# Crispy13/GeneFuseRust

Measured on NVIDIA B200. Metric: read_pairs_per_sec_matched, higher is better.
Workload: dtype u8/int64

## Files before the change

### genefuserust_b200/csrc/gf_api.cu

```cuda
#include <algorithm>
#include <chrono>
#include <cstdlib>
#include <condition_variable>
#include <cstring>
#include <mutex>
#include <thread>

#include "gf_internal.h"

static thread_local std::string g_last_error;
void gf_set_error(const std::string& msg) { g_last_error = msg; }

__global__ void k_fill_uniform(uint64_t* off, uint32_t* pko, uint64_t base, uint32_t len, uint64_t n) {
    const uint64_t i = (uint64_t)blockIdx.x * blockDim.x + threadIdx.x;
    if (i <= n) off[i] = base + i * len;
    if (i < n) pko[i] = (uint32_t)(i * 2u * ((len + 31u) >> 5));
}

namespace {

constexpr uint64_t CHUNK_TARGET_BYTES = 192ull << 20;

int fail(int code, const std::string& msg) {
    gf_set_error(msg);
// ... 33 lines not shown
        uint64_t mx = 0;
        bool b = false;
        for (uint64_t i = n * t / nt; i < n * (t + 1) / nt; i++) {
            const uint64_t a = off1[i], e = off1[i + 1];
            b |= e < a;
            mx = std::max(mx, e - a);
            if (off2) {
                const uint64_t a2 = off2[i], e2 = off2[i + 1];
                b |= e2 < a2;
                mx = std::max(mx, e2 - a2);
            }
        }
        part[t] = mx;
        bad[t] = b;
    };
    if (nt == 1) work(0);
    else {
        std::vector<std::thread> th;
        for (unsigned t = 0; t < nt; t++) th.emplace_back(work, t);
        for (auto& x : th) x.join();
    }
    uint64_t mx = 0;
    for (unsigned t = 0; t < nt; t++) {
        if (bad[t]) return fail(GF_E_INVALID, "offsets are not ascending");
        mx = std::max(mx, part[t]);
    }
    if (mx > limit) return fail(GF_E_INVALID, "a read is longer than the kernel capacity (max_len hint too small, or > 1024 bases)");
    *max_len = mx;
    return GF_OK;
}

void destroy_handle(gf_index* idx) {
    if (!idx) return;
    cudaSetDevice(idx->device);
    if (idx->busy && idx->ev_busy) cudaEventSynchronize(idx->ev_busy);
    if (idx->stream) cudaStreamSynchronize(idx->stream);
    if (idx->copy_stream) cudaStreamSynchronize(idx->copy_stream);
    cudaFree(idx->d_table);
    cudaFree(idx->d_dupes);
    cudaFree(idx->d_gene_ascii);
    cudaFree(idx->d_gene_start);
    cudaFree(idx->d_gene_len);
    cudaFree(idx->d_gene_rev);
    cudaFree(idx->d_planes);
    cudaFree(idx->d_filter);
    cudaFree(idx->d_granule);
    idx->ws_survivors.release();
    idx->ws_counters.release();
    idx->ws_gtbl.release();
    idx->ws_seq_words.release();
    idx->ws_seq_meta.release();
    idx->ws_seq_seed.release();
    idx->ws_seq_lists.release();
    idx->fq[0].release();
    idx->fq[1].release();
    idx->bgzf_comp[0].release(); idx->bgzf_comp[1].release();
    idx->bgzf_members[0].release(); idx->bgzf_members[1].release();
    idx->bgzf_status.release();
    for (auto& s : idx->stage) {
        s.seq1.release(); s.qual1.release(); s.off1.release();
        s.seq2.release(); s.qual2.release(); s.off2.release();
        s.out.release(); s.nout.release(); s.out2.release(); s.keys.release();
        for (int m = 0; m < 2; m++) {
            s.pk[m].release(); s.pko[m].release(); s.pkx[m].release(); s.pxo[m].release();
        }
        if (s.copied) cudaEventDestroy(s.copied);
        if (s.done) cudaEventDestroy(s.done);
    }
    for (auto& ps : idx->pack_set) {
        for (int m = 0; m < 2; m++) { ps.h_pk[m].release(); ps.h_pko[m].release(); ps.h_pkx[m].release(); ps.h_pxo[m].release(); }
        if (ps.copied) cudaEventDestroy(ps.copied);
    }
    if (idx->h_slots) cudaFreeHost(idx->h_slots);
    for (cudaEvent_t e : {idx->ev_start, idx->ev_end, idx->ev_ingest})
        if (e) cudaEventDestroy(e);
    for (GfChunkEvents& ce : idx->chunk_events)
        for (cudaEvent_t e : ce.e)
            if (e) cudaEventDestroy(e);
    if (idx->stream) cudaStreamDestroy(idx->stream);
    if (idx->copy_stream) cudaStreamDestroy(idx->copy_stream);
    if (idx->ev_busy) cudaEventDestroy(idx->ev_busy);
    delete idx;
}

}

extern "C" {

const char* gf_last_error(void) { return g_last_error.c_str(); }
int gf_abi_version(void) { return GF_ABI_VERSION; }

int gf_device_count(void) {
    int n = 0;
    if (cudaGetDeviceCount(&n) != cudaSuccess) {
        cudaGetLastError();
        return 0;
    }
    return n;
}

void gf_default_params(gf_params* p) {
    p->skip_key_dup_threshold = 5;
    p->major_gene_key_requirement = 40;
    p->minor_gene_key_requirement = 20;
    p->mismatch_threshold = 10;
    p->deletion_threshold = 50;
// ... 1137 lines not shown
```

### genefuserust_b200/csrc/gf_internal.h

```cpp
#pragma once
#include <cuda_runtime.h>

#include <mutex>
#include <string>
#include <vector>

#include "../../include/genefuse_gpu.h"
#include "gf_device.cuh"
#include "gf_pack.h"

void gf_set_error(const std::string& msg);

#define GF_CUDA_TRY(expr)                                                                              \
    do {                                                                                               \
        cudaError_t _e = (expr);                                                                       \
        if (_e != cudaSuccess) {                                                                       \
            gf_set_error(std::string(#expr) + " failed: " + cudaGetErrorString(_e) + " (" + __FILE__ + \
                         ":" + std::to_string(__LINE__) + ")");                                        \
            return GF_E_CUDA;                                                                          \
        }                                                                                              \
    } while (0)

struct GfBuf {
    void* p = nullptr;
// ... 77 lines not shown

struct GfFastqTable {
    uint64_t n_records = 0;
    uint32_t max_len = 0;
    GfBuf nl, s, e, qs;
    GfBuf cnt, off, tmp;
    void release() { nl.release(); s.release(); e.release(); qs.release(); cnt.release(); off.release(); tmp.release(); }
};

struct GfChunkEvents {
    cudaEvent_t e[6] = {nullptr, nullptr, nullptr, nullptr, nullptr, nullptr};
};

struct GfBgzfMember {
    uint64_t in_off;
    uint64_t out_off;
    uint32_t clen, isize, crc, pad;
};
int gf_bgzf_inflate_device(const uint8_t* d_comp, const GfBgzfMember* d_members, uint32_t n, uint8_t* d_text, unsigned int* d_status,
                           cudaStream_t st);
struct GfFastqMembers {
    const uint8_t* comp = nullptr;
    uint64_t comp_bytes = 0;
    const GfBgzfMember* members = nullptr;
    uint32_t n_members = 0;
    uint64_t text_bytes = 0;
};

struct gf_index {
    int device = 0;
    gf_params params{};
    GfDevIndex dev{};
    gf_index_info info{};
    uint32_t n_genes = 0;
    std::vector<uint32_t> gene_start, gene_len;

    void *d_table = nullptr, *d_dupes = nullptr, *d_gene_ascii = nullptr, *d_gene_start = nullptr,
         *d_gene_len = nullptr, *d_gene_rev = nullptr, *d_planes = nullptr, *d_filter = nullptr, *d_granule = nullptr;

    std::mutex mu;
    cudaStream_t stream = nullptr, copy_stream = nullptr;
    cudaEvent_t ev_busy = nullptr;
    bool busy = false;
    cudaEvent_t ev_start = nullptr, ev_end = nullptr;
    cudaEvent_t ev_ingest = nullptr;
    std::vector<GfChunkEvents> chunk_events;
    uint32_t n_chunks_timed = 0;
    bool split_events = false;
    bool ev_valid = false;

    GfBuf ws_survivors, ws_counters, ws_gtbl;
    GfFastqTable fq[2];
    GfBuf ws_seq_words, ws_seq_meta, ws_seq_seed, ws_seq_lists;
    GfStage stage[GF_STAGES];
    GfPackSet pack_set[GF_PACK_SETS];
    GfBuf bgzf_comp[2], bgzf_members[2], bgzf_status;
    GfHostSlot* h_slots = nullptr;
    bool stats_pending = false;
    uint64_t pending_pairs = 0;
    gf_map_stats stats{};
    unsigned long long launches = 0;
    int sm_count = 148;
    uint32_t out_mode = 0;
};

int gf_build_index_device(gf_index* idx, const gf_gene_span* genes, uint32_t n_genes);
int gf_lookup_device(gf_index* idx, const uint32_t* kmers, uint64_t n, gf_lookup* out);

size_t gf_scan_tmp_elems(uint64_t n);
cudaError_t gf_exclusive_scan_u32(const uint32_t* in, uint32_t* out, uint64_t n, uint32_t* tmp, cudaStream_t st);

int gf_fastq_parse_device(const uint8_t* d_text, uint64_t bytes, GfFastqTable* out, cudaStream_t st, bool final_chunk = true);
int gf_map_fastq_text(gf_index* idx, const uint8_t* fq1, uint64_t bytes1, const uint8_t* fq2, uint64_t bytes2, bool final_chunk,
                      gf_match* out, uint64_t out_cap, uint64_t* n_out, uint64_t* n_records, uint64_t consumed[2],
                      const GfFastqMembers* members = nullptr );
int gf_fastq_fetch_text(gf_index* idx, int k, uint64_t from, uint64_t len, uint8_t* dst);

struct GfDevBatch {
    uint64_t n;
    const uint8_t *seq1, *qual1, *seq2, *qual2;
    const uint64_t *s1, *e1, *qs1, *s2, *e2, *qs2;
    uint64_t base1, base2;
    uint64_t bytes1, bytes2;
    uint64_t pair_base;
    uint32_t max_len;
    const uint32_t *pk1 = nullptr, *pk2 = nullptr;
    const uint32_t *pko1 = nullptr, *pko2 = nullptr;
    const uint32_t *pkx1 = nullptr, *pkx2 = nullptr;
    const uint32_t *pxo1 = nullptr, *pxo2 = nullptr;
};
int gf_map_device_batch(gf_index* idx, const GfDevBatch& b, gf_match* d_out, uint64_t out_cap,
                        unsigned long long* d_n_out, cudaStream_t stream, GfChunkEvents* ev, bool first,
                        gf_index* store_owner = nullptr);
int gf_map_device_batches(gf_index* const* hs, uint32_t nh, const GfDevBatch& b, gf_match* const* d_outs, uint64_t out_cap,
                          unsigned long long* const* d_n_outs, cudaStream_t stream);
int gf_finish_records_device(gf_index* idx, const gf_match* d_in, const unsigned long long* d_n_in, uint64_t in_cap,
                             gf_match* d_out2, unsigned long long* d_keys, unsigned long long* d_n_out2, uint32_t mode,
                             cudaStream_t stream);
int gf_fast_merge_device(gf_index* idx, const GfDevBatch& b, gf_merge_info* d_out, cudaStream_t stream);
int gf_adjust_break_device(gf_index* idx, const uint8_t* d_bytes, const gf_break_ref* d_refs, const gf_break_job* d_jobs,
                           uint64_t n_jobs, gf_break_out* d_out, unsigned int* d_n_undefined, cudaStream_t stream);
```

### genefuserust_b200/csrc/gf_map.cu

```cuda
#include <climits>
#include <cstdlib>
#include <cstdio>

#include "gf_internal.h"
#include "gf_swar.cuh"

namespace {

#define FULL 0xFFFFFFFFu
using swar::zero_bytes;

__device__ __forceinline__ uint32_t fsr(const uint32_t* plane, uint32_t bitpos) {
    uint32_t w = bitpos >> 5;
    return __funnelshift_r(plane[w], plane[w + 1], bitpos & 31u);
}
__device__ __forceinline__ uint32_t lowmask(int nbits) {
    return nbits >= 32 ? 0xFFFFFFFFu : ((1u << nbits) - 1u);
}
__device__ __forceinline__ bool record_ok(uint64_t s, uint64_t e, uint64_t base, uint64_t bytes, int max_len) {
    if (e < s || e - s > (uint64_t)max_len || s < base) return false;
    return bytes == 0 || (s - base <= bytes && e - s <= bytes - (s - base));
}

template <int MAXW>
// ... 1230 lines not shown

int gf_map_device_batch(gf_index* idx, const GfDevBatch& b, gf_match* d_out, uint64_t out_cap,
                        unsigned long long* d_n_out, cudaStream_t st, GfChunkEvents* ev, bool first, gf_index* store_owner) {
    const bool record_events = ev != nullptr;
    if (ev)
        for (cudaEvent_t& e : ev->e)
            if (!e) GF_CUDA_TRY(cudaEventCreate(&e));
    const bool paired = b.seq2 != nullptr;
    if (b.n > 0xFFFFFFFFull) {
        gf_set_error("batch too large (n > 2^32-1 pairs): split it");
        return GF_E_LIMIT;
    }
    const uint64_t surv_cap64 = (paired ? 2 : 1) * b.n + 1;
    const uint32_t surv_cap = (uint32_t)(surv_cap64 > 0xFFFFFFFFull ? 0xFFFFFFFFull : surv_cap64);
    GF_CUDA_TRY(idx->ws_survivors.reserve(sizeof(uint2) * (size_t)surv_cap));
    GF_CUDA_TRY(idx->ws_counters.reserve(sizeof(GfMapCounters)));
    GfMapCounters* d_cnt = idx->ws_counters.as<GfMapCounters>();
    if (first) {
        GF_CUDA_TRY(cudaMemsetAsync(d_cnt, 0, sizeof(GfMapCounters), st));
        GF_CUDA_TRY(cudaMemsetAsync(d_n_out, 0, sizeof(unsigned long long), st));
    } else {
        k_roll_counters<<<1, 1, 0, st>>>(d_cnt, d_n_out, out_cap);
    }
    if (record_events) { GF_CUDA_TRY(cudaEventRecord(ev->e[0], st)); idx->split_events = false; }

    const int need_major = (idx->params.major_gene_key_requirement + 1) / 2;
    const int need_minor = (idx->params.minor_gene_key_requirement + 1) / 2;
    ScreenParams sp;
    sp.ix = idx->dev;
    sp.b = b;
    sp.survivors = idx->ws_survivors.as<uint2>();
    sp.survivors_cap = surv_cap;
    sp.counters = d_cnt;
    sp.need_total = need_major + need_minor;
    sp.need_minor = need_minor;

    if (b.n) {
        const int threads = 256, warps = threads / 32;
        const bool small = b.max_len != 0 && b.max_len <= 256;
        const size_t smem = (small ? sizeof(ScreenWarp<8>) : sizeof(ScreenWarp<32>)) * warps;
        const int blocks_per_sm = 3;
        uint64_t want = (b.n + warps - 1) / warps;
        unsigned grid = (unsigned)std::min<uint64_t>(want, (uint64_t)idx->sm_count * blocks_per_sm);
        if (small) {
            const bool w5 = b.max_len <= 160;
            const int NW3 = w5 ? split::SL<5>::NW3 : split::SL<8>::NW3;
            const uint32_t cap = surv_cap;
            const size_t groups = ((size_t)cap + 31) / 32;
            gf_index* own = store_owner ? store_owner : idx;
            if (!store_owner) {
                GF_CUDA_TRY(idx->ws_seq_words.reserve(groups * NW3 * 32 * sizeof(uint32_t)));
                GF_CUDA_TRY(idx->ws_seq_meta.reserve((size_t)cap * sizeof(uint4)));
            }
            GF_CUDA_TRY(idx->ws_seq_seed.reserve((size_t)cap * sizeof(uint2)));
            GF_CUDA_TRY(idx->ws_seq_lists.reserve((size_t)cap * sizeof(uint32_t) + 64));
            split::SeqStore ss;
            ss.words = own->ws_seq_words.as<uint32_t>();
            ss.meta = own->ws_seq_meta.as<uint4>();
            ss.seed = idx->ws_seq_seed.as<uint2>();
            ss.counters = idx->ws_seq_lists.as<unsigned int>();
            ss.list = idx->ws_seq_lists.as<uint32_t>() + 16;
            ss.cap = cap;
            GF_CUDA_TRY(cudaMemsetAsync(ss.counters, 0, 64, st));
            if (store_owner) {
                const unsigned int* oc = store_owner->ws_seq_lists.as<unsigned int>();
                GF_CUDA_TRY(cudaMemcpyAsync(ss.counters, oc, sizeof(unsigned int), cudaMemcpyDeviceToDevice, st));
                GF_CUDA_TRY(cudaMemcpyAsync(ss.counters + 5, oc + 5, sizeof(unsigned int), cudaMemcpyDeviceToDevice, st));
            }
            split::PrepParams pp;
            pp.b = b;
            pp.st = ss;
            pp.counters = d_cnt;
            const size_t psm = sizeof(uint32_t) * tpp::WARPS * (w5 ? tpp::Lay<5>::NWORDS : tpp::Lay<8>::NWORDS) * 32;
            const uint64_t want_b = (b.n + tpp::WARPS * 32 - 1) / (tpp::WARPS * 32);
#define GF_LAUNCH_PREP2(WW, PE, PK)                                                        \
    do {                                                                                   \
        GF_CUDA_TRY(set_smem(split::k_prep<WW, PE, PK>, psm));                             \
        const unsigned pgrid = (unsigned)std::min<uint64_t>(                               \
            want_b, (uint64_t)idx->sm_count * resident_blocks(split::k_prep<WW, PE, PK>, tpp::WARPS * 32, psm)); \
        split::k_prep<WW, PE, PK><<<pgrid, tpp::WARPS * 32, psm, st>>>(pp);                \
    } while (0)
#define GF_LAUNCH_PREP(WW, PE) do { if (b.pk1) GF_LAUNCH_PREP2(WW, PE, true); else GF_LAUNCH_PREP2(WW, PE, false); } while (0)
            if (!store_owner) {
                if (w5) { if (paired) GF_LAUNCH_PREP(5, true); else GF_LAUNCH_PREP(5, false); }
                else { if (paired) GF_LAUNCH_PREP(8, true); else GF_LAUNCH_PREP(8, false); }
            }
#undef GF_LAUNCH_PREP2
#undef GF_LAUNCH_PREP
            if (record_events) GF_CUDA_TRY(cudaEventRecord(ev->e[1], st));
            split::SeedParams sdp;
            sdp.ix = idx->dev;
            sdp.st = ss;
            sdp.need_total = sp.need_total;
            sdp.need_minor = sp.need_minor;
            split::ClassParams cp;
            cp.ix = idx->dev;
            cp.st = ss;
            cp.survivors = sp.survivors;
            cp.survivors_cap = sp.survivors_cap;
            cp.counters = d_cnt;
            cp.need_total = sp.need_total;
            cp.need_minor = sp.need_minor;
            const unsigned smc = (unsigned)idx->sm_count;
#define GF_EV(k) do { if (record_events) GF_CUDA_TRY(cudaEventRecord(ev->e[k], st)); } while (0)
#define GF_LAUNCH_CLASSES(WW)                                                                                         \
    do {                                                                                                              \
        split::k_seed<WW><<<smc * resident_blocks(split::k_seed<WW>, 256, 0), 256, 0, st>>>(sdp);                     \
        GF_EV(2);                                                                                                     \
        split::k_diag<WW><<<smc * resident_blocks(split::k_diag<WW>, 256, 0), 256, 0, st>>>(cp);                      \
        GF_EV(3);                                                                                                     \
        split::k_scan<WW><<<smc * resident_blocks(split::k_scan<WW>, 256, 0), 256, 0, st>>>(cp);                      \
    } while (0)
            if (w5) GF_LAUNCH_CLASSES(5); else GF_LAUNCH_CLASSES(8);
#undef GF_LAUNCH_CLASSES
#undef GF_EV
            if (record_events) idx->split_events = true;
            idx->launches += 3;
        } else {
            GF_CUDA_TRY(set_smem(k_screen<32, true>, smem));
            GF_CUDA_TRY(set_smem(k_screen<32, false>, smem));
            if (paired) k_screen<32, true><<<grid, threads, smem, st>>>(sp);
            else k_screen<32, false><<<grid, threads, smem, st>>>(sp);
        }
        GF_CUDA_TRY(cudaGetLastError());
        idx->launches++;
    }
    if (record_events) GF_CUDA_TRY(cudaEventRecord(ev->e[4], st));

    if (b.n) {
        const bool ex_small = b.max_len != 0 && b.max_len <= 256;
        const size_t ex_smem = (ex_small ? sizeof(ExactWarpSmall) : sizeof(ExactWarpLarge)) * EX_WARPS;
        const int ex_gslots = ex_small ? ExactWarpSmall::GLOBAL_SLOTS : ExactWarpLarge::GLOBAL_SLOTS;
        if (ex_small) GF_CUDA_TRY(set_smem(k_exact<ExactWarpSmall>, ex_smem));
        else GF_CUDA_TRY(set_smem(k_exact<ExactWarpLarge>, ex_smem));
        const unsigned ex_res = ex_small ? resident_blocks(k_exact<ExactWarpSmall>, EX_WARPS * 32, ex_smem)
                                         : resident_blocks(k_exact<ExactWarpLarge>, EX_WARPS * 32, ex_smem);
        const unsigned ex_grid = (unsigned)idx->sm_count * std::min(ex_res, 10u);
        const size_t n_ex_warps = (size_t)ex_grid * EX_WARPS;
        static_assert(sizeof(long long) == 8, "");
        GfBuf& gt = idx->ws_gtbl;
        GF_CUDA_TRY(gt.reserve(n_ex_warps * ex_gslots * (sizeof(long long) + sizeof(int))));
        ExactParams ep;
        ep.ix = idx->dev;
        ep.b = b;
        ep.survivors = idx->ws_survivors.as<uint2>();
        ep.survivors_cap = surv_cap;
        ep.counters = d_cnt;
        ep.out = d_out;
        ep.out_cap = out_cap;
        ep.n_out = d_n_out;
        ep.gtbl_keys = gt.as<long long>();
        ep.gtbl_cnt = (int*)(gt.as<long long>() + n_ex_warps * ex_gslots);
        if (ex_small) k_exact<ExactWarpSmall><<<ex_grid, EX_WARPS * 32, ex_smem, st>>>(ep);
        else k_exact<ExactWarpLarge><<<ex_grid, EX_WARPS * 32, ex_smem, st>>>(ep);
        GF_CUDA_TRY(cudaGetLastError());
        VerifyParams vp;
        vp.ix = idx->dev;
        vp.b = b;
        vp.counters = d_cnt;
        vp.out = d_out;
        vp.out_cap = out_cap;
        vp.n_out = d_n_out;
        if (ex_small)
            k_verify<544><<<(unsigned)idx->sm_count * std::min(resident_blocks(k_verify<544>, VF_WARPS * 32, 0), 8u), VF_WARPS * 32, 0, st>>>(vp);
        else
            k_verify<EX_SEQ_CAP><<<(unsigned)idx->sm_count * std::min(resident_blocks(k_verify<EX_SEQ_CAP>, VF_WARPS * 32, 0), 8u), VF_WARPS * 32, 0, st>>>(vp);
        GF_CUDA_TRY(cudaGetLastError());
        idx->launches += 2;
    }
    if (record_events) GF_CUDA_TRY(cudaEventRecord(ev->e[5], st));
    return GF_OK;
}

int gf_map_device_batches(gf_index* const* hs, uint32_t nh, const GfDevBatch& b, gf_match* const* d_outs, uint64_t out_cap,
                          unsigned long long* const* d_n_outs, cudaStream_t st) {
    const bool small = b.max_len != 0 && b.max_len <= 256;
    const uint64_t per_pair = (small ? 2ull * ((b.max_len <= 160 ? split::SL<5>::NW3 : split::SL<8>::NW3) * 4 + 16 + 8) : 0ull) + 8 + 16;
    uint64_t chunk = std::max<uint64_t>(1u << 20, (5ull << 30) / per_pair);
    if (const char* e = getenv("GF_DEVICE_CHUNK_PAIRS")) { long long v = atoll(e); if (v >= 1024) chunk = (uint64_t)v; }
    const uint64_t n_chunks = b.n ? (b.n + chunk - 1) / chunk : 1;
    const uint64_t per = b.n ? (b.n + n_chunks - 1) / n_chunks : 0;
    for (uint32_t h = 0; h < nh; h++) {
        if (hs[h]->chunk_events.size() < n_chunks) hs[h]->chunk_events.resize(n_chunks);
        hs[h]->n_chunks_timed = (uint32_t)n_chunks;
    }
    for (uint64_t c = 0; c < n_chunks; c++) {
        const uint64_t lo = c * per, hi = std::min(b.n, lo + per);
        GfDevBatch cb = b;
        cb.n = hi - lo;
        cb.s1 += lo; cb.e1 += lo; cb.qs1 += lo;
        if (cb.s2) { cb.s2 += lo; cb.e2 += lo; cb.qs2 += lo; }
        cb.pair_base = b.pair_base + lo;
        for (uint32_t h = 0; h < nh; h++) {
            int rc = gf_map_device_batch(hs[h], cb, d_outs[h], out_cap, d_n_outs[h], st, &hs[h]->chunk_events[c], c == 0,
                                         h ? hs[0] : nullptr);
            if (rc != GF_OK) return rc;
        }
    }
    return GF_OK;
}

int gf_finish_records_device(gf_index* idx, const gf_match* d_in, const unsigned long long* d_n_in, uint64_t in_cap,
                             gf_match* d_out2, unsigned long long* d_keys, unsigned long long* d_n_out2, uint32_t mode,
                             cudaStream_t st) {
    GF_CUDA_TRY(cudaMemsetAsync(d_n_out2, 0, sizeof(unsigned long long), st));
    k_finish<<<(unsigned)idx->sm_count, 256, 0, st>>>(d_in, d_n_in, in_cap, d_out2, d_keys, d_n_out2, idx->n_genes, mode);
    GF_CUDA_TRY(cudaGetLastError());
    idx->launches++;
    return GF_OK;
}

int gf_fast_merge_device(gf_index* idx, const GfDevBatch& b, gf_merge_info* d_out, cudaStream_t st) {
    if (!b.n) return GF_OK;
    GF_CUDA_TRY(idx->ws_counters.reserve(sizeof(GfMapCounters)));
    GF_CUDA_TRY(cudaMemsetAsync(idx->ws_counters.p, 0, sizeof(GfMapCounters), st));
    if (b.max_len != 0 && b.max_len <= 256) {
        const bool w5 = b.max_len <= 160;
        const size_t tsm = sizeof(uint32_t) * tpp::WARPS * (w5 ? tpp::Lay<5>::NWORDS : tpp::Lay<8>::NWORDS) * 32;
        unsigned tgrid = (unsigned)std::min<uint64_t>((b.n + tpp::WARPS * 32 - 1) / (tpp::WARPS * 32), (uint64_t)idx->sm_count * 3);
        if (w5) {
            GF_CUDA_TRY(set_smem(tpp::k_merge_only_tpp<5>, tsm));
            tpp::k_merge_only_tpp<5><<<tgrid, tpp::WARPS * 32, tsm, st>>>(b, d_out, idx->ws_counters.as<GfMapCounters>());
        } else {
            GF_CUDA_TRY(set_smem(tpp::k_merge_only_tpp<8>, tsm));
            tpp::k_merge_only_tpp<8><<<tgrid, tpp::WARPS * 32, tsm, st>>>(b, d_out, idx->ws_counters.as<GfMapCounters>());
        }
        GF_CUDA_TRY(cudaGetLastError());
        return GF_OK;
    }
    const int threads = 256, warps = 8;
    const size_t smem = sizeof(ScreenWarp<32>) * warps;
    GF_CUDA_TRY(set_smem(k_merge_only<32>, smem));
// ... 24 lines not shown
```

### genefuserust_b200/csrc/gf_screen_split.cuh

```cuda
#pragma once

namespace split {

using tpp::Col;
using tpp::Lay;

#ifndef GF_STORE_STREAMING
#define GF_STORE_STREAMING 1
#endif
template <class T>
__device__ __forceinline__ T st_ld(const T* p) {
#if GF_STORE_STREAMING
    return __ldcs(p);
#else
    return *p;
#endif
}
template <class T>
__device__ __forceinline__ void st_st(T* p, T v) {
#if GF_STORE_STREAMING
    __stcs(p, v);
#else
    *p = v;
#endif
// ... 138 lines not shown
                            const int fp = f ? fix1 : fix0;
                            if (fp >= 0 && (fp >> 5) == k) {
                                const uint32_t bit = 1u << (fp & 31);
                                lo = (lo & ~bit) | (c(Lay<W>::R1LO, k) & bit);
                                hi = (hi & ~bit) | (c(Lay<W>::R1HI, k) & bit);
                                v = (v & ~bit) | (c(Lay<W>::R1V, k) & bit);
                            }
                        }
                    }
                }
                st_st(&w[(size_t)k * 32], lo); st_st(&w[(size_t)(NW + k) * 32], hi); st_st(&w[(size_t)(2 * NW + k) * 32], v);
            }
            const uint32_t info = merged ? (0u | ((uint32_t)olen << 2) | ((uint32_t)diff << 14)) : 1u;
            st_st(&P.st.meta[slot0], make_uint4((uint32_t)p, info, (uint32_t)len0, 0u));
            c_seq++;
            c_merged += merged ? 1u : 0u;
            c_bytes += (unsigned)len0;
            c_probes += (unsigned)(len0 >= 16 ? ((len0 - 16) >> 1) + 1 : 0);
        }
        if (nseq == 2) {
            uint32_t* w = slot_words<W>(P.st, slot0 + 1u);
            const int nw = (len2 + 31) >> 5;
            for (int k = 0; k <= nw; k++) {
                uint32_t lo = 0, hi = 0, v = 0;
                if (k < nw) {
                    const int pos = len2 - 32 * k - 32;
                    v = __brev(c.win(Lay<W>::VCS, pos));
                    lo = ~__brev(c.win(Lay<W>::C2LO, pos)) & v;
                    hi = __brev(c.win(Lay<W>::C2HI, pos)) & v;
                }
                st_st(&w[(size_t)k * 32], lo); st_st(&w[(size_t)(NW + k) * 32], hi); st_st(&w[(size_t)(2 * NW + k) * 32], v);
            }
            st_st(&P.st.meta[slot0 + 1u], make_uint4((uint32_t)p, 2u, (uint32_t)len2, 0u));
            c_seq++;
            c_bytes += (unsigned)len2;
            c_probes += (unsigned)(len2 >= 16 ? ((len2 - 16) >> 1) + 1 : 0);
        }
        __syncwarp();
    }
    c_seq = __reduce_add_sync(FULL, c_seq);
    c_merged = __reduce_add_sync(FULL, c_merged);
    c_probes = __reduce_add_sync(FULL, c_probes);
    c_bytes = __reduce_add_sync(FULL, c_bytes);
    if (lane == 0) {
        if (c_seq) atomicAdd(&P.counters->n_sequences, (unsigned long long)c_seq);
        if (c_probes) atomicAdd(&P.counters->n_probes, (unsigned long long)c_probes);
        if (c_bytes) atomicAdd(&P.counters->seq_bytes, (unsigned long long)c_bytes);
        if (c_merged) atomicAdd(&P.counters->n_merged, (unsigned long long)c_merged);
    }
    err = __reduce_or_sync(FULL, err);
    if (err && lane == 0) atomicOr(&P.counters->error_flags, err);
}

struct SeedParams {
    GfDevIndex ix;
    SeqStore st;
    int need_total, need_minor;
};
template <int W>
__global__ void __launch_bounds__(256) k_seed(SeedParams P) {
    constexpr int NW = SL<W>::NW;
    const uint32_t lane = gf_lane();
    const uint32_t n_short = min(P.st.counters[0], P.st.cap), n_long = min(P.st.counters[5], P.st.cap - n_short);
    const uint32_t n_slots = n_short + n_long;
    const unsigned long long pol = make_policy_keep();
    const uint32_t stride = gridDim.x * blockDim.x;
    const uint32_t wib = threadIdx.x >> 5;
    __shared__ uint32_t cls_cnt[8][2], cls_base[8][2];
    for (uint32_t b0 = blockIdx.x * blockDim.x; b0 < n_slots; b0 += stride) {
        const uint32_t vi = b0 + threadIdx.x;
        const uint32_t s = vi < n_short ? vi : P.st.cap - n_long + (vi - n_short);
        bool have = vi < n_slots, seeded = false;
        uint32_t seed_val = GF_EMPTY_VAL, seed_i = 0;
        if (have) {
            const uint32_t* col = slot_words<W>(P.st, s);
            uint32_t plo[4], phi[4], pv[4];
#pragma unroll
            for (int j = 0; j < 4; j++) {
                plo[j] = st_ld(&col[(size_t)j * 32]); phi[j] = st_ld(&col[(size_t)(NW + j) * 32]); pv[j] = st_ld(&col[(size_t)(2 * NW + j) * 32]);
            }
            const uint4 m = st_ld(&P.st.meta[s]);
            const int len = (int)m.z;
            const int nprobe = len >= 16 ? ((len - 16) >> 1) + 1 : 0;
            if (nprobe == 0 && P.need_total > 0) have = false;
            if (have && nprobe > 0) {
                uint32_t key[8], okm = 0;
#pragma unroll
                for (int j = 0; j < 4; j++) {
                    key[2 * j] = (phi[j] << 16) | (plo[j] & 0xFFFFu);
                    key[2 * j + 1] = (phi[j] & 0xFFFF0000u) | (plo[j] >> 16);
                    if (32 * j + 16 <= len && (pv[j] & 0xFFFFu) == 0xFFFFu) okm |= 1u << (2 * j);
                    if (32 * j + 32 <= len && (pv[j] >> 16) == 0xFFFFu) okm |= 2u << (2 * j);
                }
                if (okm) {
                    const uint32_t t0 = (uint32_t)__ffs(okm) - 1u;
                    uint32_t k0 = key[0];
#pragma unroll
                    for (int t = 1; t < 8; t++) if (t0 == (uint32_t)t) k0 = key[t];
                    tpp::prefetch_l2(P.ix.table + 2ull * gf_home_bucket(k0, P.ix.bucket_shift));
                }
                unsigned long long fw[8];
#pragma unroll
                for (int t = 0; t < 8; t++) {
                    fw[t] = 0;
                    if ((okm >> t) & 1u) fw[t] = ldg_filter(P.ix.filter + gf_filter_word(key[t], P.ix.filter_words), pol);
                }
                uint32_t pm = 0;
#pragma unroll
                for (int t = 0; t < 8; t++) {
                    uint32_t al, ah;
                    gf_filter_masks(key[t], &al, &ah);
                    const uint32_t wl = (uint32_t)fw[t], wh = (uint32_t)(fw[t] >> 32);
                    if (((okm >> t) & 1u) && (wl & al) == al && (wh & ah) == ah) pm |= 1u << t;
                }
                seed_i = pm | (okm << 8);
                while (pm) {
                    const int t = __ffs(pm) - 1;
                    pm &= pm - 1u;
                    uint32_t kt = key[0];
#pragma unroll
                    for (int u = 1; u < 8; u++) if (t == u) kt = key[u];
                    const uint32_t val = gf_table_find(P.ix, kt);
                    if (val != GF_EMPTY_VAL && (val >> 30) == GF_KIND_UNIQUE) {
                        seed_val = val;
                        seed_i = 16u * (uint32_t)t;
                        seeded = true;
                        break;
                    }
                }
            }
            if (have) st_st(&P.st.seed[s], make_uint2(seed_val, seed_i));
        }
        const int cls = have ? (seeded ? 0 : 1) : -1;
        const uint32_t m0 = __ballot_sync(FULL, cls == 0), m1 = __ballot_sync(FULL, cls == 1);
        if (lane == 0) { cls_cnt[wib][0] = (uint32_t)__popc(m0); cls_cnt[wib][1] = (uint32_t)__popc(m1); }
        __syncthreads();
        if (threadIdx.x < 2) {
            uint32_t tot = 0;
#pragma unroll
            for (int w = 0; w < 8; w++) tot += cls_cnt[w][threadIdx.x];
            uint32_t bb = tot ? atomicAdd(&P.st.counters[1 + threadIdx.x], tot) : 0u;
#pragma unroll
            for (int w = 0; w < 8; w++) { cls_base[w][threadIdx.x] = bb; bb += cls_cnt[w][threadIdx.x]; }
        }
        __syncthreads();
        if (cls == 0) st_st(&P.st.list[cls_base[wib][0] + __popc(m0 & gf_lanemask_lt())], s);
        else if (cls == 1) st_st(&P.st.list[P.st.cap - 1u - (cls_base[wib][1] + __popc(m1 & gf_lanemask_lt()))], s);
    }
}

struct ClassParams {
    GfDevIndex ix;
    SeqStore st;
    uint2* survivors;
    uint32_t survivors_cap;
    GfMapCounters* counters;
    int need_total, need_minor;
};
__device__ __forceinline__ void push_survivor(const ClassParams& P, const uint4& m) {
    uint32_t slot = atomicAdd(&P.counters->n_survivors, 1u);
    if (slot < P.survivors_cap) P.survivors[slot] = make_uint2(m.x, m.y);
    else atomicOr(&P.counters->error_flags, 2u);
}
template <int W>
__global__ void __launch_bounds__(256) k_scan(ClassParams P) {
    constexpr int NW = SL<W>::NW;
    const unsigned long long pol = make_policy_keep();
    const GfDevIndex& ix = P.ix;
    const int need_major = P.need_total - P.need_minor;
    const uint32_t n = P.st.counters[2];
    for (uint32_t t = blockIdx.x * blockDim.x + threadIdx.x; t < n; t += gridDim.x * blockDim.x) {
        const uint32_t s = st_ld(&P.st.list[P.st.cap - 1u - t]);
        const uint4 m = st_ld(&P.st.meta[s]);
        const int len = (int)m.z, nch = (len + 31) >> 5;
        const uint32_t* col = slot_words<W>(P.st, s);
        uint32_t lo = st_ld(&col[0]), hi = st_ld(&col[(size_t)NW * 32]), v = st_ld(&col[(size_t)2 * NW * 32]);
        const uint32_t pre = st_ld(&P.st.seed[s]).y, pre_valid = (pre >> 8) & 0xFFu;
        int Pn = __popc(pre & 0xFFu);
        bool dead = false;
#pragma unroll 1
        for (int k = 0; k < nch && !dead; k++) {
            const uint32_t nlo = st_ld(&col[(size_t)(k + 1) * 32]), nhi = st_ld(&col[(size_t)(NW + k + 1) * 32]), nv = st_ld(&col[(size_t)(2 * NW + k + 1) * 32]);
            uint32_t om = run16(v, nv) & 0x55555555u;
            if (k < 4) om &= ~0x00010001u;
            const int beyond = len - 16 - 32 * (k + 1);
            const int rem_after = (beyond >= 0 ? (beyond >> 1) + 1 : 0) - (k < 3 ? __popc(pre_valid >> (2 * (k + 1))) : 0);
// ... 147 lines not shown
```

### genefuserust_b200/csrc/gf_screen_tpp.cuh

```cuda
#pragma once

namespace tpp {

using swar::block16;
using swar::fill16;

template <int W>
struct Lay {
    static constexpr int R1LO = 0, R1HI = R1LO + W + 1, R1V = R1HI + W + 1, R1N = R1V + W + 1;
    static constexpr int C2LO = R1N + W + 1, C2HI = C2LO + W + 1, C2V = C2HI + W + 1, VCS = C2V + W + 1;
    static constexpr int NWORDS = VCS + W + 1;
};
constexpr int WARPS = 4;

struct Col {
    uint32_t* base;
    __device__ __forceinline__ uint32_t& operator()(int arr, int k) const { return base[(arr + k) * 32]; }
    __device__ __forceinline__ uint32_t fs(int arr, uint32_t bitpos) const {
        uint32_t w = bitpos >> 5;
        return __funnelshift_r(base[(arr + (int)w) * 32], base[(arr + (int)w + 1) * 32], bitpos & 31u);
    }
    __device__ __forceinline__ uint32_t win(int arr, int pos) const {
        if (pos >= 0) return fs(arr, (uint32_t)pos);
        if (pos > -32) return base[arr * 32] << (-pos);
        return 0u;
    }
};

__device__ __forceinline__ uint32_t load4_guarded(const uint8_t* p, const uint8_t* lo, const uint8_t* hi) {
    if (p >= lo && p + 4 <= hi) return __ldg(reinterpret_cast<const uint32_t*>(p));
    uint32_t w = 0;
    for (int t = 0; t < 4; t++)
        if (p + t >= lo && p + t < hi) w |= (uint32_t)__ldg(p + t) << (8 * t);
    return w;
}
__device__ __forceinline__ void prefetch_l2(const void* p) { asm volatile("prefetch.global.L2 [%0];" ::"l"(p)); }

__device__ __noinline__ uint4 load16_slow(const uint8_t* p, const uint8_t* lo, const uint8_t* hi) {
    return make_uint4(load4_guarded(p, lo, hi), load4_guarded(p + 4, lo, hi), load4_guarded(p + 8, lo, hi),
                      load4_guarded(p + 12, lo, hi));
}
__device__ __forceinline__ void load32_span(const uint8_t* p, bool span_inside, const uint8_t* lo, const uint8_t* hi,
                                            unsigned long long pol_stream, uint4* a, uint4* b) {
    if (span_inside) {
        asm volatile("ld.global.nc.L1::no_allocate.L2::cache_hint.v8.u32 {%0,%1,%2,%3,%4,%5,%6,%7}, [%8], %9;"
                     : "=r"(a->x), "=r"(a->y), "=r"(a->z), "=r"(a->w), "=r"(b->x), "=r"(b->y), "=r"(b->z), "=r"(b->w)
                     : "l"(p), "l"(pol_stream));
        return;
    }
    *a = load16_slow(p, lo, hi);
    *b = load16_slow(p + 16, lo, hi);
}
__device__ __forceinline__ unsigned long long make_policy_normal() {
    unsigned long long pol;
    asm volatile("createpolicy.fractional.L2::evict_normal.b64 %0, 1.0;" : "=l"(pol));
    return pol;
}
__device__ __forceinline__ unsigned long long make_policy_stream() {
    unsigned long long pol;
    asm volatile("createpolicy.fractional.L2::evict_first.b64 %0, 1.0;" : "=l"(pol));
    return pol;
}

__device__ __forceinline__ uint32_t tailmask(int rem) {
    return rem >= 32 ? 0xFFFFFFFFu : (rem > 0 ? (1u << rem) - 1u : 0u);
}

template <int W>
__device__ __forceinline__ void convert_r1(const Col& c, const uint8_t* seq, int len, const uint8_t* lo, const uint8_t* hi,
                                           unsigned long long pol_stream) {
    const uint32_t a = (uint32_t)((uintptr_t)seq & 31u);
    const uint8_t* bp = seq - a;
    const int nu = len + (int)a;
    const int nwords = len > 0 ? (nu + 31) >> 5 : 0;
    uint32_t plo = 0, phi = 0, pv = 0, pn = 0;
    const bool inside = bp >= lo && bp + 32 * nwords <= hi;
    uint4 A = fill16(), B = fill16();
    if (nwords > 0) load32_span(bp, inside, lo, hi, pol_stream, &A, &B);
#pragma unroll 1
    for (int m = 0; m < nwords; m++) {
        uint4 nA = fill16(), nB = fill16();
        bp += 32;
        if (m + 1 < nwords) load32_span(bp, inside, lo, hi, pol_stream, &nA, &nB);
        uint32_t l0, h0, v0, n0, l1, h1, v1, n1;
        block16<false>(A, &l0, &h0, &v0, &n0);
        block16<false>(B, &l1, &h1, &v1, &n1);
        const uint32_t ulo = __byte_perm(l0, l1, 0x5410u), uhi = __byte_perm(h0, h1, 0x5410u);
        const uint32_t uv = __byte_perm(v0, v1, 0x5410u), un = __byte_perm(n0, n1, 0x5410u);
        if (m > 0) {
// ... 213 lines not shown
```

Measured before the change: 1.989 billion.

## Split seed kernel into probe, bucket-binned lookup, and list passes

The single seed kernel is split into three kernels. The probe pass runs the filter and scatters the first filter hit of each read into bins keyed by hash-table home bucket. The lookup pass then walks the bins in order so hash-table accesses are localized in cache. A final pass builds the seeded and unseeded class lists from the stored seeds. This aims to cut random hash-table traffic, at the cost of two extra launches, a bin workspace with atomics, and a new cap on chunk size.

```diff
diff --git a/genefuserust_b200/csrc/gf_api.cu b/genefuserust_b200/csrc/gf_api.cu
--- a/genefuserust_b200/csrc/gf_api.cu
+++ b/genefuserust_b200/csrc/gf_api.cu
@@ -109,6 +109,7 @@
     idx->ws_seq_meta.release();
     idx->ws_seq_seed.release();
     idx->ws_seq_lists.release();
+    idx->ws_seq_bins.release();
     idx->fq[0].release();
     idx->fq[1].release();
     idx->bgzf_comp[0].release(); idx->bgzf_comp[1].release();
diff --git a/genefuserust_b200/csrc/gf_internal.h b/genefuserust_b200/csrc/gf_internal.h
--- a/genefuserust_b200/csrc/gf_internal.h
+++ b/genefuserust_b200/csrc/gf_internal.h
@@ -153,6 +153,7 @@
     GfBuf ws_survivors, ws_counters, ws_gtbl;
     GfFastqTable fq[2];
     GfBuf ws_seq_words, ws_seq_meta, ws_seq_seed, ws_seq_lists;
+    GfBuf ws_seq_bins;
     GfStage stage[GF_STAGES];
     GfPackSet pack_set[GF_PACK_SETS];
     GfBuf bgzf_comp[2], bgzf_members[2], bgzf_status;
diff --git a/genefuserust_b200/csrc/gf_map.cu b/genefuserust_b200/csrc/gf_map.cu
--- a/genefuserust_b200/csrc/gf_map.cu
+++ b/genefuserust_b200/csrc/gf_map.cu
@@ -1306,8 +1306,18 @@
                 GF_CUDA_TRY(idx->ws_seq_words.reserve(groups * NW3 * 32 * sizeof(uint32_t)));
                 GF_CUDA_TRY(idx->ws_seq_meta.reserve((size_t)cap * sizeof(uint4)));
             }
+            if (cap >= (1u << split::SEED_SLOT_BITS)) {
+                gf_set_error("device chunk too large for the seed bins (>= 2^28 pairs): lower GF_DEVICE_CHUNK_PAIRS");
+                return GF_E_LIMIT;
+            }
             GF_CUDA_TRY(idx->ws_seq_seed.reserve((size_t)cap * sizeof(uint2)));
             GF_CUDA_TRY(idx->ws_seq_lists.reserve((size_t)cap * sizeof(uint32_t) + 64));
+            const uint32_t bucket_bits = 32u - idx->dev.bucket_shift, bin_lg = split::seed_bin_lg(bucket_bits);
+            const uint32_t n_bins = 1u << (bucket_bits - bin_lg);
+            const uint32_t bin_mean = (uint32_t)(((uint64_t)cap + n_bins - 1) / n_bins);
+            const uint32_t bin_cap = bin_mean + bin_mean / 8 + 64;
+            const size_t bin_cnt_bytes = ((size_t)n_bins * sizeof(unsigned int) + 255) & ~(size_t)255;
+            GF_CUDA_TRY(idx->ws_seq_bins.reserve(bin_cnt_bytes + (size_t)n_bins * bin_cap * sizeof(uint2)));
             split::SeqStore ss;
             ss.words = own->ws_seq_words.as<uint32_t>();
             ss.meta = own->ws_seq_meta.as<uint4>();
@@ -1316,6 +1326,7 @@
             ss.list = idx->ws_seq_lists.as<uint32_t>() + 16;
             ss.cap = cap;
             GF_CUDA_TRY(cudaMemsetAsync(ss.counters, 0, 64, st));
+            GF_CUDA_TRY(cudaMemsetAsync(idx->ws_seq_bins.p, 0, bin_cnt_bytes, st));
             if (store_owner) {
                 const unsigned int* oc = store_owner->ws_seq_lists.as<unsigned int>();
                 GF_CUDA_TRY(cudaMemcpyAsync(ss.counters, oc, sizeof(unsigned int), cudaMemcpyDeviceToDevice, st));
@@ -1345,8 +1356,12 @@
             split::SeedParams sdp;
             sdp.ix = idx->dev;
             sdp.st = ss;
+            sdp.bin_cnt = idx->ws_seq_bins.as<unsigned int>();
+            sdp.bins = reinterpret_cast<uint2*>(idx->ws_seq_bins.as<unsigned char>() + bin_cnt_bytes);
+            sdp.bin_cap = bin_cap;
+            sdp.n_bins = n_bins;
+            sdp.bin_lg = bin_lg;
             sdp.need_total = sp.need_total;
-            sdp.need_minor = sp.need_minor;
             split::ClassParams cp;
             cp.ix = idx->dev;
             cp.st = ss;
@@ -1359,7 +1374,9 @@
 #define GF_EV(k) do { if (record_events) GF_CUDA_TRY(cudaEventRecord(ev->e[k], st)); } while (0)
 #define GF_LAUNCH_CLASSES(WW)                                                                                         \
     do {                                                                                                              \
-        split::k_seed<WW><<<smc * resident_blocks(split::k_seed<WW>, 256, 0), 256, 0, st>>>(sdp);                     \
+        split::k_seed_probe<WW><<<smc * resident_blocks(split::k_seed_probe<WW>, 256, 0), 256, 0, st>>>(sdp);         \
+        split::k_seed_lookup<WW><<<smc * resident_blocks(split::k_seed_lookup<WW>, 256, 0), 256, 0, st>>>(sdp);       \
+        split::k_seed_lists<<<smc * resident_blocks(split::k_seed_lists, 256, 0), 256, 0, st>>>(sdp);                 \
         GF_EV(2);                                                                                                     \
         split::k_diag<WW><<<smc * resident_blocks(split::k_diag<WW>, 256, 0), 256, 0, st>>>(cp);                      \
         GF_EV(3);                                                                                                     \
@@ -1369,7 +1386,7 @@
 #undef GF_LAUNCH_CLASSES
 #undef GF_EV
             if (record_events) idx->split_events = true;
-            idx->launches += 3;
+            idx->launches += 5;
         } else {
             GF_CUDA_TRY(set_smem(k_screen<32, true>, smem));
             GF_CUDA_TRY(set_smem(k_screen<32, false>, smem));
@@ -1429,9 +1446,10 @@
 int gf_map_device_batches(gf_index* const* hs, uint32_t nh, const GfDevBatch& b, gf_match* const* d_outs, uint64_t out_cap,
                           unsigned long long* const* d_n_outs, cudaStream_t st) {
     const bool small = b.max_len != 0 && b.max_len <= 256;
-    const uint64_t per_pair = (small ? 2ull * ((b.max_len <= 160 ? split::SL<5>::NW3 : split::SL<8>::NW3) * 4 + 16 + 8) : 0ull) + 8 + 16;
+    const uint64_t per_pair = (small ? 2ull * ((b.max_len <= 160 ? split::SL<5>::NW3 : split::SL<8>::NW3) * 4 + 16 + 8 + 9) : 0ull) + 8 + 16;
     uint64_t chunk = std::max<uint64_t>(1u << 20, (5ull << 30) / per_pair);
     if (const char* e = getenv("GF_DEVICE_CHUNK_PAIRS")) { long long v = atoll(e); if (v >= 1024) chunk = (uint64_t)v; }
+    if (small) chunk = std::min<uint64_t>(chunk, (1ull << (split::SEED_SLOT_BITS - 1)) - 1);
     const uint64_t n_chunks = b.n ? (b.n + chunk - 1) / chunk : 1;
     const uint64_t per = b.n ? (b.n + n_chunks - 1) / n_chunks : 0;
     for (uint32_t h = 0; h < nh; h++) {
diff --git a/genefuserust_b200/csrc/gf_screen_split.cuh b/genefuserust_b200/csrc/gf_screen_split.cuh
--- a/genefuserust_b200/csrc/gf_screen_split.cuh
+++ b/genefuserust_b200/csrc/gf_screen_split.cuh
@@ -214,86 +214,146 @@
     if (err && lane == 0) atomicOr(&P.counters->error_flags, err);
 }
 
+constexpr uint32_t SEED_BIN_LG = 9;
+constexpr uint32_t SEED_MIN_BINS_LG = 11;
+constexpr uint32_t SEED_SLOT_BITS = 29;
+constexpr uint32_t SEED_DROPPED = 0xFFFFFFFFu;
+
 struct SeedParams {
     GfDevIndex ix;
     SeqStore st;
-    int need_total, need_minor;
+    uint2* bins;
+    unsigned int* bin_cnt;
+    uint32_t bin_cap, n_bins, bin_lg;
+    int need_total;
 };
+__host__ __device__ inline uint32_t seed_bin_lg(uint32_t bucket_bits) {
+    return bucket_bits > SEED_MIN_BINS_LG + SEED_BIN_LG ? SEED_BIN_LG : (bucket_bits > SEED_MIN_BINS_LG ? bucket_bits - SEED_MIN_BINS_LG : 0u);
+}
+
+__device__ __forceinline__ void seed_keys(const uint32_t plo[4], const uint32_t phi[4], uint32_t key[8]) {
+#pragma unroll
+    for (int j = 0; j < 4; j++) {
+        key[2 * j] = (phi[j] << 16) | (plo[j] & 0xFFFFu);
+        key[2 * j + 1] = (phi[j] & 0xFFFF0000u) | (plo[j] >> 16);
+    }
+}
+__device__ __forceinline__ bool seed_first_unique(const GfDevIndex& ix, const uint32_t key[8], uint32_t pm, uint2* sd) {
+    while (pm) {
+        const int t = __ffs(pm) - 1;
+        pm &= pm - 1u;
+        uint32_t kt = key[0];
+#pragma unroll
+        for (int u = 1; u < 8; u++) if (t == u) kt = key[u];
+        const uint32_t val = gf_table_find(ix, kt);
+        if (val != GF_EMPTY_VAL && (val >> 30) == GF_KIND_UNIQUE) {
+            *sd = make_uint2(val, 16u * (uint32_t)t);
+            return true;
+        }
+    }
+    return false;
+}
+__device__ __forceinline__ uint32_t seed_slot(const SeqStore& st, uint32_t vi, uint32_t n_short, uint32_t n_long) {
+    return vi < n_short ? vi : st.cap - n_long + (vi - n_short);
+}
+
 template <int W>
-__global__ void __launch_bounds__(256) k_seed(SeedParams P) {
+__global__ void __launch_bounds__(256) k_seed_probe(SeedParams P) {
     constexpr int NW = SL<W>::NW;
+    const uint32_t n_short = min(P.st.counters[0], P.st.cap), n_long = min(P.st.counters[5], P.st.cap - n_short);
+    const uint32_t n_slots = n_short + n_long;
+    const unsigned long long pol = make_policy_keep();
+    for (uint32_t vi = blockIdx.x * blockDim.x + threadIdx.x; vi < n_slots; vi += gridDim.x * blockDim.x) {
+        const uint32_t s = seed_slot(P.st, vi, n_short, n_long);
+        const uint32_t* col = slot_words<W>(P.st, s);
+        uint32_t plo[4], phi[4], pv[4];
+#pragma unroll
+        for (int j = 0; j < 4; j++) {
+            plo[j] = st_ld(&col[(size_t)j * 32]); phi[j] = st_ld(&col[(size_t)(NW + j) * 32]); pv[j] = st_ld(&col[(size_t)(2 * NW + j) * 32]);
+        }
+        const int len = (int)st_ld(&P.st.meta[s]).z;
+        const int nprobe = len >= 16 ? ((len - 16) >> 1) + 1 : 0;
+        uint2 sd = make_uint2(GF_EMPTY_VAL, 0u);
+        if (nprobe == 0) {
+            if (P.need_total > 0) sd.y = SEED_DROPPED;
+        } else {
+            uint32_t key[8], okm = 0;
+            seed_keys(plo, phi, key);
+#pragma unroll
+            for (int j = 0; j < 4; j++) {
+                if (32 * j + 16 <= len && (pv[j] & 0xFFFFu) == 0xFFFFu) okm |= 1u << (2 * j);
+                if (32 * j + 32 <= len && (pv[j] >> 16) == 0xFFFFu) okm |= 2u << (2 * j);
+            }
+            unsigned long long fw[8];
+#pragma unroll
+            for (int t = 0; t < 8; t++) {
+                fw[t] = 0;
+                if ((okm >> t) & 1u) fw[t] = ldg_filter(P.ix.filter + gf_filter_word(key[t], P.ix.filter_words), pol);
+            }
+            uint32_t pm = 0;
+#pragma unroll
+            for (int t = 0; t < 8; t++) {
+                uint32_t al, ah;
+                gf_filter_masks(key[t], &al, &ah);
+                const uint32_t wl = (uint32_t)fw[t], wh = (uint32_t)(fw[t] >> 32);
+                if (((okm >> t) & 1u) && (wl & al) == al && (wh & ah) == ah) pm |= 1u << t;
+            }
+            sd.y = pm | (okm << 8);
+            if (pm) {
+                const uint32_t t0 = (uint32_t)__ffs(pm) - 1u;
+                uint32_t k0 = key[0];
+#pragma unroll
+                for (int t = 1; t < 8; t++) if (t0 == (uint32_t)t) k0 = key[t];
+                const uint32_t bin = gf_home_bucket(k0, P.ix.bucket_shift) >> P.bin_lg;
+                const uint32_t e = atomicAdd(&P.bin_cnt[bin], 1u);
+                if (e < P.bin_cap) st_st(&P.bins[(size_t)bin * P.bin_cap + e], make_uint2(k0, s | (t0 << SEED_SLOT_BITS)));
+                else seed_first_unique(P.ix, key, pm, &sd);
+            }
+        }
+        st_st(&P.st.seed[s], sd);
+    }
+}
+
+template <int W>
+__global__ void __launch_bounds__(256) k_seed_lookup(SeedParams P) {
+    constexpr int NW = SL<W>::NW;
+    const uint32_t n = P.n_bins * P.bin_cap;
+    for (uint32_t v = blockIdx.x * blockDim.x + threadIdx.x; v < n; v += gridDim.x * blockDim.x) {
+        const uint32_t b = v / P.bin_cap, e = v - b * P.bin_cap;
+        if (e >= __ldg(&P.bin_cnt[b])) continue;
+        const uint2 en = st_ld(&P.bins[v]);
+        const uint32_t s = en.y & ((1u << SEED_SLOT_BITS) - 1u), t0 = en.y >> SEED_SLOT_BITS;
+        const uint32_t val = gf_table_find(P.ix, en.x);
+        uint2 sd = make_uint2(val, 16u * t0);
+        bool seeded = val != GF_EMPTY_VAL && (val >> 30) == GF_KIND_UNIQUE;
+        if (!seeded) {
+            const uint32_t* col = slot_words<W>(P.st, s);
+            uint32_t plo[4], phi[4], key[8];
+#pragma unroll
+            for (int j = 0; j < 4; j++) { plo[j] = st_ld(&col[(size_t)j * 32]); phi[j] = st_ld(&col[(size_t)(NW + j) * 32]); }
+            seed_keys(plo, phi, key);
+            const uint32_t pm = st_ld(&P.st.seed[s]).y & 0xFFu;
+            seeded = seed_first_unique(P.ix, key, pm & (pm - 1u), &sd);
+        }
+        if (seeded) st_st(&P.st.seed[s], sd);
+    }
+}
+
+__global__ void __launch_bounds__(256) k_seed_lists(SeedParams P) {
     const uint32_t lane = gf_lane();
     const uint32_t n_short = min(P.st.counters[0], P.st.cap), n_long = min(P.st.counters[5], P.st.cap - n_short);
     const uint32_t n_slots = n_short + n_long;
-    const unsigned long long pol = make_policy_keep();
     const uint32_t stride = gridDim.x * blockDim.x;
     const uint32_t wib = threadIdx.x >> 5;
     __shared__ uint32_t cls_cnt[8][2], cls_base[8][2];
     for (uint32_t b0 = blockIdx.x * blockDim.x; b0 < n_slots; b0 += stride) {
         const uint32_t vi = b0 + threadIdx.x;
-        const uint32_t s = vi < n_short ? vi : P.st.cap - n_long + (vi - n_short);
-        bool have = vi < n_slots, seeded = false;
-        uint32_t seed_val = GF_EMPTY_VAL, seed_i = 0;
-        if (have) {
-            const uint32_t* col = slot_words<W>(P.st, s);
-            uint32_t plo[4], phi[4], pv[4];
-#pragma unroll
-            for (int j = 0; j < 4; j++) {
-                plo[j] = st_ld(&col[(size_t)j * 32]); phi[j] = st_ld(&col[(size_t)(NW + j) * 32]); pv[j] = st_ld(&col[(size_t)(2 * NW + j) * 32]);
-            }
-            const uint4 m = st_ld(&P.st.meta[s]);
-            const int len = (int)m.z;
-            const int nprobe = len >= 16 ? ((len - 16) >> 1) + 1 : 0;
-            if (nprobe == 0 && P.need_total > 0) have = false;
-            if (have && nprobe > 0) {
-                uint32_t key[8], okm = 0;
-#pragma unroll
-                for (int j = 0; j < 4; j++) {
-                    key[2 * j] = (phi[j] << 16) | (plo[j] & 0xFFFFu);
-                    key[2 * j + 1] = (phi[j] & 0xFFFF0000u) | (plo[j] >> 16);
-                    if (32 * j + 16 <= len && (pv[j] & 0xFFFFu) == 0xFFFFu) okm |= 1u << (2 * j);
-                    if (32 * j + 32 <= len && (pv[j] >> 16) == 0xFFFFu) okm |= 2u << (2 * j);
-                }
-                if (okm) {
-                    const uint32_t t0 = (uint32_t)__ffs(okm) - 1u;
-                    uint32_t k0 = key[0];
-#pragma unroll
-                    for (int t = 1; t < 8; t++) if (t0 == (uint32_t)t) k0 = key[t];
-                    tpp::prefetch_l2(P.ix.table + 2ull * gf_home_bucket(k0, P.ix.bucket_shift));
-                }
-                unsigned long long fw[8];
-#pragma unroll
-                for (int t = 0; t < 8; t++) {
-                    fw[t] = 0;
-                    if ((okm >> t) & 1u) fw[t] = ldg_filter(P.ix.filter + gf_filter_word(key[t], P.ix.filter_words), pol);
-                }
-                uint32_t pm = 0;
-#pragma unroll
-                for (int t = 0; t < 8; t++) {
-                    uint32_t al, ah;
-                    gf_filter_masks(key[t], &al, &ah);
-                    const uint32_t wl = (uint32_t)fw[t], wh = (uint32_t)(fw[t] >> 32);
-                    if (((okm >> t) & 1u) && (wl & al) == al && (wh & ah) == ah) pm |= 1u << t;
-                }
-                seed_i = pm | (okm << 8);
-                while (pm) {
-                    const int t = __ffs(pm) - 1;
-                    pm &= pm - 1u;
-                    uint32_t kt = key[0];
-#pragma unroll
-                    for (int u = 1; u < 8; u++) if (t == u) kt = key[u];
-                    const uint32_t val = gf_table_find(P.ix, kt);
-                    if (val != GF_EMPTY_VAL && (val >> 30) == GF_KIND_UNIQUE) {
-                        seed_val = val;
-                        seed_i = 16u * (uint32_t)t;
-                        seeded = true;
-                        break;
-                    }
-                }
-            }
-            if (have) st_st(&P.st.seed[s], make_uint2(seed_val, seed_i));
-        }
-        const int cls = have ? (seeded ? 0 : 1) : -1;
+        const uint32_t s = seed_slot(P.st, vi, n_short, n_long);
+        int cls = -1;
+        if (vi < n_slots) {
+            const uint2 sd = st_ld(&P.st.seed[s]);
+            if (sd.y != SEED_DROPPED) cls = sd.x != GF_EMPTY_VAL ? 0 : 1;
+        }
         const uint32_t m0 = __ballot_sync(FULL, cls == 0), m1 = __ballot_sync(FULL, cls == 1);
         if (lane == 0) { cls_cnt[wib][0] = (uint32_t)__popc(m0); cls_cnt[wib][1] = (uint32_t)__popc(m1); }
         __syncthreads();
diff --git a/genefuserust_b200/csrc/gf_screen_tpp.cuh b/genefuserust_b200/csrc/gf_screen_tpp.cuh
--- a/genefuserust_b200/csrc/gf_screen_tpp.cuh
+++ b/genefuserust_b200/csrc/gf_screen_tpp.cuh
@@ -34,7 +34,6 @@
         if (p + t >= lo && p + t < hi) w |= (uint32_t)__ldg(p + t) << (8 * t);
     return w;
 }
-__device__ __forceinline__ void prefetch_l2(const void* p) { asm volatile("prefetch.global.L2 [%0];" ::"l"(p)); }
 
 __device__ __noinline__ uint4 load16_slow(const uint8_t* p, const uint8_t* lo, const uint8_t* hi) {
     return make_uint4(load4_guarded(p, lo, hi), load4_guarded(p + 4, lo, hi), load4_guarded(p + 8, lo, hi),
```

Result: slower. 1.795 billion (median of 6 runs) (-9.8%).
